# qwerfdsaplking/SATrans

Hardware: AMD Instinct MI355X
Metric: training samples/sec (AliCCP-shaped, emb=32, 3L/4H, meta_mode=QK) (higher is better)
Workload: dtype f32; 1 GPU; BASELINE configs[1]: AliCCP-shaped SATrans training step, 19 fields, 6,571,961 table rows (841 MB fp32), uniform ids, dropout on, dense-Adam+L2 semantics over all rows; batch_per_gpu=8192, global_batch=8192, embedding_dim=32, layers=3, heads=4, fields=19, parallelism=dp1

## Files before the change

include/satrans_hip.h:

```cpp
#ifndef SATRANS_HIP_H
#define SATRANS_HIP_H

#include <stdint.h>

#ifdef __cplusplus
extern "C" {
#endif

#define SATRANS_ABI_VERSION 7

#define SATRANS_OK 0
#define SATRANS_E_BADARG (-1)
#define SATRANS_E_UNSUPPORTED (-2)
#define SATRANS_E_LAUNCH (-3)
#define SATRANS_E_WORKSPACE (-4)

#define SATRANS_ID_F32 0
#define SATRANS_ID_I32 1
#define SATRANS_ID_I64 2

#define SATRANS_META_Q 1
#define SATRANS_META_K 2
#define SATRANS_RELU_OUT 4
#define SATRANS_NO_RES 8
// ... 697 lines not shown
int satrans_layer_bwd_head_supported(const satrans_layer_desc* d, const satrans_head_desc* h);
int satrans_stack_fwd_bf16_head(int n, const satrans_layer_desc* const* descs, const satrans_head_desc* h, void* stream);
int64_t satrans_layer_bwd_head_scratch_floats(const satrans_layer_desc* d, int n_dense);
int satrans_layer_bwd_head(const satrans_layer_desc* d, const satrans_head_desc* h, float* dx, float* slabs, float* g_wq,
                           float* g_wk, float* g_wv, float* g_wo, float* g_ln, float* g_lnq, float* g_lnk, float* g_tab_q,
                           float* g_tab_k, void* stream);

typedef struct satrans_layer_grads {
    float *g_wq, *g_wk, *g_wv, *g_wo, *g_ln, *g_lnq, *g_lnk, *g_tab_q, *g_tab_k;
} satrans_layer_grads;
int satrans_layer_bwd_deferred_supported(const satrans_layer_desc* d);
int satrans_layer_bwd_launch(const satrans_layer_desc* d, const float* dy, float* dx, float* slabs, void* stream);
int satrans_layer_bwd_head_launch(const satrans_layer_desc* d, const satrans_head_desc* h, float* dx, float* slabs, void* stream);
int satrans_layer_bwd_reduce(int n, const satrans_layer_desc* const* h_descs, float* const* h_slabs,
                             const satrans_layer_grads* h_grads, const satrans_head_desc* head, void* stream);

#define SATRANS_OPT_SGD 1
#define SATRANS_OPT_ADAGRAD 2
#define SATRANS_OPT_RMSPROP 3
int satrans_optim_flat(int kind, float* p, const float* g, float* state, int64_t n, float lr, float alpha, float eps, void* stream);
int64_t satrans_head_scratch_floats(int B, int FD, int n_dense);

#define SATRANS_ADAM_EXACT 0
#define SATRANS_ADAM_FAST  1
typedef struct satrans_adam_hparams {
    float lr_over_bc1;
    float bc2_sqrt;
    float beta1, beta2, eps;
    float l2;
    int32_t arith;
// ... 113 lines not shown
```

satrans_amd/csrc/embed_adam.hip:

```cpp
#include <algorithm>
#include <cstdlib>
#include <cstring>

#include <rocprim/rocprim.hpp>

#include "common.h"

namespace satrans {

constexpr int kChunk = 16;
constexpr int kStreamBlock = 256;
constexpr int kStreamBlocks = 2048;

struct AdamK {
    float neg_step, w1, beta2, w2, eps, l2x2, l2;
    double rbc2;
    float rbc2f;
    int fast;
};

__host__ inline AdamK make_adamk(const satrans_adam_hparams& h) {
    AdamK k;
    k.neg_step = -h.lr_over_bc1;
    k.rbc2 = 1.0 / (double)h.bc2_sqrt;
// ... 110 lines not shown
    if (i >= n) return;
    keys[i] = (uint32_t)rows[i];
    pos[i] = (int32_t)i;
}

__global__ void mark_heads_kernel(const int32_t* __restrict__ sorted_rows, int64_t n, uint32_t* __restrict__ touched) {
    const int64_t i = (int64_t)blockIdx.x * blockDim.x + threadIdx.x;
    if (i >= n) return;
    const uint32_t r = (uint32_t)sorted_rows[i];
    if (i > 0 && (uint32_t)sorted_rows[i - 1] == r) return;
    atomicOr(&touched[r >> 5], 1u << (r & 31));
}

constexpr int kSuper = 16;
template <int LPR>
__device__ __forceinline__ void touched_super_body(int64_t group, int q, int64_t chunks, const float4* partial, const int32_t* info,
                                                   const int32_t* trail_row, float4* partial2, int32_t* info2, int32_t* trail_row2,
                                                   float4* done_sum, int32_t* done_row) {
    const int64_t c0 = group * kSuper;
    if (c0 < chunks) {
        const int64_t c1 = min(chunks, c0 + (int64_t)kSuper);
        int f[kSuper];
        float4 lead[kSuper];
#pragma unroll
        for (int u = 0; u < kSuper; ++u) f[u] = c0 + u < c1 ? info[c0 + u] : 0;
#pragma unroll
        for (int u = 0; u < kSuper; ++u)
            lead[u] = c0 + u < c1 ? partial[((c0 + u) * 2 + 0) * LPR + q] : make_float4(0.f, 0.f, 0.f, 0.f);
        bool open = f[0] & 2, is_lead = open;
        int flags2 = open ? 2 : 0;
        int32_t row = -1;
        float4 acc = make_float4(0.f, 0.f, 0.f, 0.f);
#pragma unroll
        for (int u = 0; u < kSuper; ++u) {
            const int64_t c = c0 + u;
            int32_t ended = -1;
            if (f[u] & 2) {
                const float4 g = lead[u];
                acc.x += g.x; acc.y += g.y; acc.z += g.z; acc.w += g.w;
                if (f[u] & 4) {
                    if (is_lead) {
                        partial2[(group * 2 + 0) * LPR + q] = acc;
                        flags2 |= 4;
                    } else {
                        done_sum[c * LPR + q] = acc;
                        ended = row;
                    }
                    open = false;
                    is_lead = false;
                }
            }
            if (f[u] & 1) {
                acc = partial[(c * 2 + 1) * LPR + q];
                row = trail_row[c];
                open = true;
                is_lead = false;
            }
            if (q == 0 && c < c1) done_row[c] = ended;
        }
        if (open) {
            if (is_lead) {
                partial2[(group * 2 + 0) * LPR + q] = acc;
            } else {
                partial2[(group * 2 + 1) * LPR + q] = acc;
                flags2 |= 1;
                if (q == 0) trail_row2[group] = row;
            }
        }
        if (q == 0) info2[group] = flags2;
    }
}

template <int LPR>
__global__ __launch_bounds__(256) void touched_super_kernel(int64_t chunks, const float4* partial, const int32_t* info,
                                                           const int32_t* trail_row, float4* partial2, int32_t* info2,
                                                           int32_t* trail_row2, float4* done_sum, int32_t* done_row) {
    __builtin_amdgcn_s_setprio(3);
    touched_super_body<LPR>(((int64_t)blockIdx.x * 256 + threadIdx.x) / LPR, threadIdx.x % LPR, chunks, partial, info, trail_row, partial2,
                            info2, trail_row2, done_sum, done_row);
}

template <int LPR>
__global__ __launch_bounds__(256) void touched_chunks_kernel(float4* __restrict__ P, float4* __restrict__ M,
                                                            float4* __restrict__ V, const int32_t* __restrict__ sorted_rows,
                                                            const int32_t* __restrict__ src, int64_t n,
                                                            const float4* __restrict__ gemb, float4* partial,
                                                            int32_t* info, int32_t* trail_row,
                                                            float4* __restrict__ rowsum, int32_t* __restrict__ head_of,
                                                            float4* partial2, int32_t* info2, int32_t* trail_row2,
                                                            float4* done_sum, int32_t* done_row) {
    __builtin_amdgcn_s_setprio(3);
    const int64_t group = ((int64_t)blockIdx.x * 256 + threadIdx.x) / LPR;
    const int q = threadIdx.x % LPR;
    const int64_t start = group * kChunk;
    if (start < n) {
        int64_t head = start;
        const int64_t end = min(n, start + (int64_t)kChunk);
        const int32_t prev_row = start > 0 ? sorted_rows[start - 1] : -1;
        const int32_t next_row = end < n ? sorted_rows[end] : -1;
        int32_t cur = sorted_rows[start];
        bool begins = cur != prev_row;
        int flags = 0;
        float4 acc = make_float4(0.f, 0.f, 0.f, 0.f);
        auto flush = [&](bool ends) {
            const bool complete = begins && ends;
            if (q == 0) head_of[head] = complete ? 1 : 0;
            if (complete) {
                rowsum[head * LPR + q] = acc;
            } else if (!begins) {
                partial[(group * 2 + 0) * LPR + q] = acc;
                flags |= 2 | (ends ? 4 : 0);
            } else {
                partial[(group * 2 + 1) * LPR + q] = acc;
                flags |= 1;
                if (q == 0) trail_row[group] = cur;
            }
        };
        constexpr int kBatch = 16;
        for (int64_t jb = start; jb < end; jb += kBatch) {
            int32_t r[kBatch];
            float4 g[kBatch];
#pragma unroll
            for (int u = 0; u < kBatch; ++u) {
                const int64_t j = jb + u;
                const bool ok = j < end;
                r[u] = ok ? sorted_rows[j] : -2;
                const int32_t sidx = ok ? src[j] : 0;
                g[u] = ok ? gemb[(int64_t)sidx * LPR + q] : make_float4(0.f, 0.f, 0.f, 0.f);
            }
#pragma unroll
            for (int u = 0; u < kBatch; ++u) {
                if (jb + u < end) {
                    if (r[u] != cur) {
                        flush(true);
                        cur = r[u];
                        begins = true;
                        head = jb + u;
                        acc = make_float4(0.f, 0.f, 0.f, 0.f);
                    }
                    if (q == 0 && jb + u != head) head_of[jb + u] = 0;
                    acc.x += g[u].x; acc.y += g[u].y; acc.z += g[u].z; acc.w += g[u].w;
                }
            }
        }
        flush(next_row != cur);
        if (q == 0) info[group] = flags;
    }
    constexpr int kGroups = 256 / LPR;
    if constexpr (kGroups % kSuper == 0) {
        __syncthreads();
        const int sg = threadIdx.x / LPR;
        if (sg < kGroups / kSuper)
            touched_super_body<LPR>((int64_t)blockIdx.x * (kGroups / kSuper) + sg, q, (n + kChunk - 1) / kChunk, partial, info, trail_row,
                                    partial2, info2, trail_row2, done_sum, done_row);
    }
}

template <int LPR>
__device__ __forceinline__ void touched_apply_body(int64_t bid, double* s_red, float4* __restrict__ P, float4* __restrict__ M,
                                                   float4* __restrict__ V, const int32_t* __restrict__ sorted_rows,
                                                   int64_t n, const float4* __restrict__ rowsum,
                                                   const int32_t* __restrict__ head_of, const AdamK& k,
                                                   double* __restrict__ reg_partials, float4* __restrict__ G,
                                                   int32_t* __restrict__ last, int t) {
    const int64_t j = (bid * 256 + threadIdx.x) / LPR;
    const int q = threadIdx.x % LPR;
    double reg = 0.0;
    if (j < n && head_of[j] == 1) {
        const int64_t at = (int64_t)sorted_rows[j] * LPR + q;
// ... 1356 lines not shown
```

satrans_amd/csrc/layer_fused.hip:

```cpp
#include <hip/hip_ext.h>

#include "layer_fused_common.h"

namespace satrans {

struct KernelTimer {
    static constexpr int kPairs = 512;
    struct Pair { hipEvent_t start, stop; int kind; };
    Pair pairs[kPairs];
    int made = 0, used = 0;
    bool armed = false;
    Pair* next(int kind) {
        if (!armed || used >= kPairs) return nullptr;
        if (used >= made) {
            if (hipEventCreate(&pairs[made].start) != hipSuccess || hipEventCreate(&pairs[made].stop) != hipSuccess) return nullptr;
            ++made;
        }
        pairs[used].kind = kind;
        return &pairs[used++];
    }
};
static KernelTimer g_ktimer;

#ifdef SATRANS_DIAG_FWDSAVE
// ... 1665 lines not shown
            }
            if (threadIdx.x == 0) {
                float gb = 0.f, lsum = 0.f;
                for (int ls = 0; ls < Tsamp; ++ls) { lsum += s_fin[ls]; gb += s_fin[64 + ls]; }
                prow[ncol] = gb;
                prow[ncol + 1] = lsum;
            }
        }
    }
}


#undef WGRAD
constexpr int kRG = kReduceGroups;
constexpr int kReduceMaxLayers = 8;
__device__ __forceinline__ void fused_common_reduce(const float* __restrict__ common, int G, int D, int flags, int block,
                                                    float* g_wq, float* g_wk, float* g_wv, float* g_wo, float* g_ln,
                                                    float* g_lnq, float* g_lnk) {
    __shared__ float s_a[kRG][32], s_b[kRG][32];
    const int CSZ = 4 * D * D + 6 * D, DD = D * D;
    const int lane = threadIdx.x & 31, grp = threadIdx.x >> 5;
    const int e = block * 32 + lane;
    const bool plain = !(flags & (SATRANS_GATE | SATRANS_BILINEAR));
    const bool mq = plain && (flags & SATRANS_META_Q) && g_lnq, mk = plain && (flags & SATRANS_META_K) && g_lnk;
    const bool shared = mq && mk && g_lnq == g_lnk;
    const int r = e - 4 * DD;
    const bool second = shared && r >= 2 * D && r < 4 * D;
    const int share = (G + kRG - 1) / kRG;
    const int lo = grp * share, hi = min(G, lo + share);
    float acc = 0.f, acc2 = 0.f;
    if (e < CSZ) {
#pragma unroll 4
        for (int w = lo; w < hi; ++w) {
            acc += common[(size_t)w * CSZ + e];
            if (second) acc2 += common[(size_t)w * CSZ + e + 2 * D];
        }
    }
    s_a[grp][lane] = acc;
    s_b[grp][lane] = acc2;
    __syncthreads();
    if (grp != 0 || e >= CSZ) return;
    float t = 0.f, t2 = 0.f;
    for (int k = 0; k < kRG; ++k) { t += s_a[k][lane]; t2 += s_b[k][lane]; }
    if (e < DD) { g_wq[e] += t; return; }
    if (e < 2 * DD) { g_wk[e - DD] += t; return; }
    if (e < 3 * DD) { g_wv[e - 2 * DD] += t; return; }
    if (e < 4 * DD) { g_wo[e - 3 * DD] += t; return; }
    if (r < 2 * D) { g_ln[r] += t; return; }
    if (r < 4 * D) {
        if (shared) g_lnq[r - 2 * D] += t + t2;
        else if (mq) g_lnq[r - 2 * D] += t;
        return;
    }
    if (mk && !shared) g_lnk[r - 4 * D] += t;
}

__device__ __forceinline__ void fused_records_reduce(int n_layers, const float* const* records_of, float* const* g_tab_q_of,
                                                     float* const* g_tab_k_of, const int32_t* __restrict__ seg,
                                                     int S, int T, int G, int D, int U, int H, int flags, int64_t tab_stride,
                                                     int block, int s) {
    __shared__ float s_q[kRG][32], s_k[kRG][32];
    const int TSZ = 4 * D * U, d = D / H;
    const bool gate = flags & SATRANS_GATE, bil = flags & SATRANS_BILINEAR;
    const int half = gate ? D : (bil ? D * d : 2 * D * U);
    const int lane = threadIdx.x & 31, grp = threadIdx.x >> 5;
    const int e = block * 32 + lane;
    int total = 0, pre = 0;
    for (int k = 0; k < S; ++k) {
        if (k == s) pre = total;
        total += tiles_of(seg, k, T);
    }
    const int nt = tiles_of(seg, s, T);
    if (nt == 0) return;
    const int per = (total + G - 1) / G;
    const int w_lo = pre / per, w_hi = (pre + nt - 1) / per;
    const int share = (w_hi - w_lo + kRG) / kRG;
    const int a = w_lo + grp * share, b = min(w_hi + 1, a + share);
    const bool mq = bil || (flags & SATRANS_META_Q), mk = !bil && (flags & SATRANS_META_K);
    int src_q = e, src_k = half + e;
    if (bil && e < half) {
        const int h = e / (d * d), i = (e / d) % d, j = e % d;
        src_q = (h * d + i) * D + h * d + j;
    }
    float aq[kReduceMaxLayers], ak[kReduceMaxLayers];
#pragma unroll
    for (int l = 0; l < kReduceMaxLayers; ++l) {
        aq[l] = 0.f; ak[l] = 0.f;
        if (l < n_layers && e < half) {
            const float* records = records_of[l];
#pragma unroll 4
            for (int w = a; w < b; ++w) {
                const float* rec = records + (size_t)(w + s) * TSZ;
                if (mq) aq[l] += rec[src_q];
                if (mk) ak[l] += rec[src_k];
            }
        }
    }
#pragma unroll
    for (int l = 0; l < kReduceMaxLayers; ++l) {
        if (l >= n_layers) break;
        s_q[grp][lane] = aq[l];
        s_k[grp][lane] = ak[l];
        __syncthreads();
        if (grp == 0 && e < half) {
            float tq = 0.f, tk = 0.f;
            for (int k = 0; k < kRG; ++k) { tq += s_q[k][lane]; tk += s_k[k][lane]; }
            float* g_tab_q = g_tab_q_of[l];
            float* g_tab_k = g_tab_k_of[l];
            if (mq && mk && g_tab_q == g_tab_k) {
                g_tab_q[(size_t)s * tab_stride + e] += tq + tk;
            } else {
                if (mq) g_tab_q[(size_t)s * tab_stride + e] += tq;
                if (mk) g_tab_k[(size_t)s * tab_stride + e] += tk;
            }
        }
        __syncthreads();
    }
}

__global__ __launch_bounds__(32 * kRG) void fused_reduce_kernel(const float* __restrict__ common, const float* __restrict__ records,
                                                         const int32_t* __restrict__ seg, int S, int T, int G, int D, int U,
                                                         int H, int flags, int64_t tab_stride, int common_blocks, int record_blocks,
                                                         float* g_wq, float* g_wk, float* g_wv, float* g_wo, float* g_ln,
                                                         float* g_lnq, float* g_lnk, float* g_tab_q, float* g_tab_k) {
    const int bx = blockIdx.x;
    if (bx < common_blocks) {
        fused_common_reduce(common, G, D, flags, bx, g_wq, g_wk, g_wv, g_wo, g_ln, g_lnq, g_lnk);
    } else {
        const int rb = bx - common_blocks;
        const float* recs[1] = {records};
        float *gq[1] = {g_tab_q}, *gk[1] = {g_tab_k};
        fused_records_reduce(1, recs, gq, gk, seg, S, T, G, D, U, H, flags, tab_stride, rb % record_blocks, rb / record_blocks);
    }
}

struct ReduceLayers {
    int n;
    const float* slabs[kReduceMaxLayers];
    float* g[kReduceMaxLayers][9];
};
struct ReduceHead {
    const float* partial;
    int nblk, ncol;
    float *g_w, *g_b;
    double* loss_sum;
};
__device__ __forceinline__ void head_partials_reduce(const ReduceHead& hd, int block) {
    __shared__ double s_acc[kRG][32];
    const int lane = threadIdx.x & 31, grp = threadIdx.x >> 5;
    const int c = block * 32 + lane, ncol = hd.ncol;
    const int share = (hd.nblk + kRG - 1) / kRG;
    const int lo = grp * share, hi = min(hd.nblk, lo + share);
    double acc = 0.0;
    if (c < ncol + 2) {
        if (c == ncol + 1) {
            for (int k = lo; k < hi; ++k) acc += (double)hd.partial[(size_t)k * (ncol + 2) + c];
        } else {
            float a32 = 0.f;
#pragma unroll 8
            for (int k = lo; k < hi; ++k) a32 += hd.partial[(size_t)k * (ncol + 2) + c];
            acc = (double)a32;
        }
    }
    s_acc[grp][lane] = acc;
    __syncthreads();
    if (grp != 0 || c >= ncol + 2) return;
    if (c == ncol + 1) {
        double t = 0.0;
        for (int k = 0; k < kRG; ++k) t += s_acc[k][lane];
        hd.loss_sum[0] += t;
        return;
    }
    float t = 0.f;
    for (int k = 0; k < kRG; ++k) t += (float)s_acc[k][lane];
    if (c < ncol) hd.g_w[c] += t;
    else hd.g_b[0] += t;
}
__global__ __launch_bounds__(32 * kRG) void fused_reduce_all_kernel(ReduceLayers R, ReduceHead hd, const int32_t* __restrict__ seg,
                                                             int S, int T, int G, int D, int U, int H, int flags,
                                                             int64_t tab_stride, int common_blocks, int record_blocks,
                                                             int per_layer) {
    __builtin_amdgcn_s_setprio(3);
    int bx = blockIdx.x;
    if (bx < R.n * common_blocks) {
        const int l = bx / common_blocks;
        float* const* g = R.g[l];
        fused_common_reduce(R.slabs[l], G, D, flags, bx - l * common_blocks, g[0], g[1], g[2], g[3], g[4], g[5], g[6]);
        return;
    }
    bx -= R.n * common_blocks;
    const int n_rec = per_layer - common_blocks;
    if (bx < n_rec) {
        const float* recs[kReduceMaxLayers];
        float *gq[kReduceMaxLayers], *gk[kReduceMaxLayers];
        for (int l = 0; l < R.n; ++l) {
            recs[l] = R.slabs[l] + (size_t)G * (4 * D * D + 6 * D);
            gq[l] = R.g[l][7];
            gk[l] = R.g[l][8];
        }
        fused_records_reduce(R.n, recs, gq, gk, seg, S, T, G, D, U, H, flags, tab_stride, bx % record_blocks, bx / record_blocks);
        return;
    }
    head_partials_reduce(hd, bx - n_rec);
}


static int fused_bwd_ft(const satrans_layer_desc* d) {
    if (d->D != 32 || d->H != 4) return 0;
    const bool same = d->tab_q == d->tab_k && d->lnq_g == d->lnk_g && d->lnq_b == d->lnk_b;
    const int mod = (d->flags & SATRANS_GATE) ? 1 : ((d->flags & SATRANS_BILINEAR) ? 2 : 0);
    if (mod) return same && d->F == 19 ? 19 : 0;
    return same ? (d->F == 19 ? 19 : 0) : (d->F == 15 ? 15 : 0);
}
#ifdef SATRANS_HANDOVER_LDS
static bool fused_save_rows(const satrans_layer_desc* d) { return false; }
#else
static bool fused_save_rows(const satrans_layer_desc* d) { return kAttnMfma && fused_bwd_ft(d) != 0; }
#endif
// ... 165 lines not shown
    if (fused_bwd_plan(d, p)) {
        const int64_t CSZ = 4 * (int64_t)d->D * d->D + 6 * d->D, TSZ = 4 * (int64_t)d->D * fused_width(d);
        n = std::max<int64_t>(n, (int64_t)p.G * CSZ + (int64_t)(p.G + d->S) * TSZ);
    }
    return n;
}

static int launch_fused_reduce(const satrans_layer_desc* d, const FusedBwdPlan& p, float* slabs, float* g_wq, float* g_wk,
                               float* g_wv, float* g_wo, float* g_ln, float* g_lnq, float* g_lnk, float* g_tab_q, float* g_tab_k,
                               hipStream_t stream) {
    const int D = d->D, U = fused_width(d), CSZ = 4 * D * D + 6 * D;
    float* records = slabs + (size_t)p.G * CSZ;
    const bool meta = d->flags & (SATRANS_META_Q | SATRANS_META_K | SATRANS_BILINEAR);
    const int row_elems = (d->flags & SATRANS_GATE) ? D : ((d->flags & SATRANS_BILINEAR) ? D * (D / d->H) : 2 * D * U);
    SATRANS_REQUIRE(!meta || g_tab_q, SATRANS_E_BADARG, "layer_bwd: null generated-row gradient");
    const int common_blocks = (int)ceil_div(CSZ, 32), record_blocks = (int)ceil_div(row_elems, 32);
    fused_reduce_kernel<<<(unsigned)(common_blocks + (meta ? record_blocks * d->S : 0)), 32 * kRG, 0, stream>>>(
        slabs, records, d->seg, d->S, p.T, p.G, D, U, d->H, d->flags, d->tab_stride, common_blocks, record_blocks, g_wq, g_wk, g_wv,
        g_wo, g_ln, g_lnq, g_lnk, g_tab_q, g_tab_k);
    SATRANS_CHECK_LAUNCH("fused_reduce_kernel");
    return SATRANS_OK;
}

extern "C" int satrans_layer_bwd_launch_fused(const satrans_layer_desc* d, const float* dy, float* dx, float* slabs, void* stream_) {
    hipStream_t stream = (hipStream_t)stream_;
    FusedBwdPlan p;
    SATRANS_REQUIRE(dy && dx && slabs, SATRANS_E_BADARG, "layer_bwd: null pointer");
    const bool same = d->tab_q == d->tab_k && d->lnq_g == d->lnk_g && d->lnq_b == d->lnk_b;
    int rc;
    {
    SATRANS_REQUIRE(fused_bwd_plan(d, p), SATRANS_E_UNSUPPORTED, "layer_bwd(fused): shape not built");
    SATRANS_REQUIRE((int64_t)d->B * d->F < ((int64_t)1 << 31), SATRANS_E_UNSUPPORTED, "layer_bwd(fused): B * F must stay below 2^31");
// ... 110 lines not shown
}

extern "C" int satrans_layer_bwd_head_fused(const satrans_layer_desc* d, const satrans_head_desc* h, float* dx, float* slabs,
                                            float* g_wq, float* g_wk, float* g_wv, float* g_wo, float* g_ln, float* g_lnq,
                                            float* g_lnk, float* g_tab_q, float* g_tab_k, void* stream_) {
    SATRANS_REQUIRE(g_wq && g_wk && g_wv && g_wo && g_ln && h->loss_sum && h->g_w && h->g_b, SATRANS_E_BADARG, "layer_bwd_head: null pointer");
    int rc = satrans_layer_bwd_head_launch_fused(d, h, dx, slabs, stream_);
    if (rc) return rc;
    FusedBwdPlan p;
    fused_bwd_plan(d, p, true);
    rc = launch_fused_reduce(d, p, slabs, g_wq, g_wk, g_wv, g_wo, g_ln, g_lnq, g_lnk, g_tab_q, g_tab_k, (hipStream_t)stream_);
    if (rc) return rc;
    return satrans_head_reduce_partials(h->scratch, p.G, d->F * d->D + h->n_dense, h->g_w, h->g_b, h->loss_sum, stream_);
}

extern "C" int satrans_layer_bwd_reduce_fused(int n, const satrans_layer_desc* const* descs, float* const* slabs,
                                              const satrans_layer_grads* grads, const satrans_head_desc* head, void* stream_) {
    hipStream_t stream = (hipStream_t)stream_;
    SATRANS_REQUIRE(n >= 1 && n <= kReduceMaxLayers && descs && slabs && grads, SATRANS_E_BADARG, "layer_bwd_reduce: 1..%d layers", kReduceMaxLayers);
    const satrans_layer_desc* d = descs[0];
    FusedBwdPlan p;
    SATRANS_REQUIRE(fused_bwd_plan(d, p), SATRANS_E_UNSUPPORTED, "layer_bwd_reduce: shape not built");
    const int D = d->D, U = fused_width(d), CSZ = 4 * D * D + 6 * D;
    const bool meta = d->flags & (SATRANS_META_Q | SATRANS_META_K | SATRANS_BILINEAR);
    const int row_elems = (d->flags & SATRANS_GATE) ? D : ((d->flags & SATRANS_BILINEAR) ? D * (D / d->H) : 2 * D * U);
    const int common_blocks = (int)ceil_div(CSZ, 32), record_blocks = (int)ceil_div(row_elems, 32);
    const int per_layer = common_blocks + (meta ? record_blocks * d->S : 0);
    ReduceLayers R;
    R.n = n;
    for (int l = 0; l < n; ++l) {
        const satrans_layer_desc* e = descs[l];
        FusedBwdPlan q;
        SATRANS_REQUIRE(e->B == d->B && e->F == d->F && e->D == d->D && e->U == d->U && e->H == d->H && e->S == d->S &&
                        e->flags == d->flags && e->seg == d->seg && e->tab_stride == d->tab_stride && fused_bwd_plan(e, q) &&
                        q.G == p.G && q.T == p.T, SATRANS_E_BADARG, "layer_bwd_reduce: layer %d differs from layer 0 in shape, flags or bucketing", l);
        const satrans_layer_grads& g = grads[l];
        SATRANS_REQUIRE(slabs[l] && g.g_wq && g.g_wk && g.g_wv && g.g_wo && g.g_ln && (!meta || g.g_tab_q), SATRANS_E_BADARG,
                        "layer_bwd_reduce: null pointer (layer %d)", l);
        R.slabs[l] = slabs[l];
        float* gp[9] = {g.g_wq, g.g_wk, g.g_wv, g.g_wo, g.g_ln, g.g_lnq, g.g_lnk, g.g_tab_q, g.g_tab_k};
        for (int k = 0; k < 9; ++k) R.g[l][k] = gp[k];
    }
    ReduceHead hd{};
    int head_blocks = 0;
    if (head) {
        SATRANS_REQUIRE(head->scratch && head->g_w && head->g_b && head->loss_sum, SATRANS_E_BADARG, "layer_bwd_reduce: null head pointer");
        FusedBwdPlan ph;
        SATRANS_REQUIRE(fused_bwd_plan(d, ph, true), SATRANS_E_UNSUPPORTED, "layer_bwd_reduce: fused head not built for this shape");
        hd.partial = head->scratch; hd.nblk = ph.G; hd.ncol = d->F * d->D + head->n_dense;
        hd.g_w = head->g_w; hd.g_b = head->g_b; hd.loss_sum = head->loss_sum;
        head_blocks = (int)ceil_div(hd.ncol + 2, 32);
    }
    fused_reduce_all_kernel<<<(unsigned)(n * common_blocks + (per_layer - common_blocks) + head_blocks), 32 * kRG, 0, stream>>>(
        R, hd, d->seg, d->S, p.T, p.G, D, U, d->H, d->flags, d->tab_stride, common_blocks, record_blocks, per_layer);
    SATRANS_CHECK_LAUNCH("fused_reduce_all_kernel");
    return SATRANS_OK;
}

#ifdef SATRANS_STAMPS
extern "C" int satrans_debug_read_stamps(unsigned long long* h_out, int reset) {
    if (hipMemcpyFromSymbol(h_out, HIP_SYMBOL(satrans::g_stamps), sizeof(unsigned long long) * 16) != hipSuccess) return -1;
    if (reset) {
        unsigned long long z[16] = {0};
        if (hipMemcpyToSymbol(HIP_SYMBOL(satrans::g_stamps), z, sizeof(z)) != hipSuccess) return -1;
    }
    return 0;
}
#endif

extern "C" int satrans_kernel_timing(int on) {
    const int was = satrans::g_ktimer.armed ? 1 : 0;
// ... 25 lines not shown
```

satrans_amd/native.py:

```python
from __future__ import annotations

import ctypes as C
import os
import subprocess
from typing import Optional

import torch

os.environ.setdefault("GPU_MAX_HW_QUEUES", "8")

_HERE = os.path.dirname(os.path.abspath(__file__))
LIB_PATH = os.environ.get("SATRANS_LIB_PATH") or os.path.join(_HERE, "libsatrans_hip.so")
ABI_VERSION = 7

ID_F32, ID_I32, ID_I64 = 0, 1, 2
META_Q, META_K, RELU_OUT, NO_RES, TRAIN, GATE, BILINEAR = 1, 2, 4, 8, 16, 32, 64
X_SORTED, Y_SORTED = 128, 256

_c_f32p = C.c_void_p
_vp = C.c_void_p


class LayerDesc(C.Structure):
    _fields_ = [
# ... 492 lines not shown
                                           C.POINTER(HeadDesc), _vp]),
    "satrans_head_scratch_floats": (C.c_int64, [C.c_int, C.c_int, C.c_int]),
    "satrans_head": (C.c_int, [_vp, _vp, C.c_int64, _vp, C.c_int, C.c_int, C.c_int, _vp, _vp, _vp, _vp, _vp, _vp,
                               _vp, _vp, _vp, _vp, _vp]),
"satrans_head_loss": (C.c_int, [_vp, _vp, C.c_int64, _vp, C.c_int, C.c_int, C.c_int, _vp, _vp, _vp, _vp, _vp, _vp,
                                    _vp, _vp, _vp, _vp, C.c_int, _vp]),
    "satrans_point_loss_partials": (C.c_int64, [C.c_int]),
    "satrans_point_loss": (C.c_int, [_vp, C.c_int64, _vp, C.c_int, C.c_int, C.c_int, _vp, _vp, _vp, _vp, _vp]),
    "satrans_optim_flat": (C.c_int, [C.c_int, _vp, _vp, _vp, C.c_int64, C.c_float, C.c_float, C.c_float, _vp]),
    "satrans_adam_flat": (C.c_int, [_vp, _vp, _vp, _vp, C.c_int64, C.POINTER(AdamHParams), _vp]),
    "satrans_adam_flat_sum": (C.c_int, [_vp, _vp, _vp, _vp, C.c_int64, C.POINTER(AdamHParams), _vp, C.c_int64, _vp, _vp]),
    "satrans_embed_sort_workspace_bytes": (C.c_int64, [C.c_int64, C.c_int64]),
    "satrans_embed_sort": (C.c_int, [_vp, C.c_int64, C.c_int64, _vp, _vp, _vp, _vp, C.c_int64, _vp, _vp]),
    "satrans_embed_reg_partials": (C.c_int64, [C.c_int64, C.c_int64, C.c_int]),
    "satrans_embed_partial_ws_floats": (C.c_int64, [C.c_int64, C.c_int]),
    "satrans_scenario_table_fwd": (C.c_int, [_vp, _vp, _vp, C.c_int, C.c_int, C.c_int, _vp, _vp]),
    "satrans_scenario_table_bwd_ws_floats": (C.c_int64, [C.c_int, C.c_int]),
    "satrans_scenario_table_bwd": (C.c_int, [_vp, _vp, _vp, C.c_int, C.c_int, C.c_int, _vp, _vp, _vp, _vp, _vp]),
    "satrans_scenario_inputs_fwd": (C.c_int, [C.POINTER(_vp), _vp, C.c_int, C.c_int, C.c_int, _vp, _vp, C.c_int, _vp, _vp]),
    "satrans_scenario_inputs_bwd": (C.c_int, [C.POINTER(_vp), C.POINTER(C.c_int32), _vp, C.c_int, C.c_int, C.c_int, _vp, _vp,
                                              _vp, C.c_int, _vp]),
    "satrans_scenario_relu_fwd": (C.c_int, [_vp, C.c_int64, _vp, _vp]),
    "satrans_scenario_relu_bwd": (C.c_int, [_vp, _vp, C.c_int64, _vp, _vp]),
    "satrans_embed_adam_touched": (C.c_int, [_vp, _vp, _vp, C.c_int, _vp, _vp, C.c_int64, _vp, _vp,
                                             C.POINTER(AdamHParams), _vp, _vp, C.c_int, _vp]),
    "satrans_embed_adam_untouched": (C.c_int, [_vp, _vp, _vp, C.c_int64, C.c_int64, C.c_int, _vp, C.POINTER(AdamHParams),
                                               _vp, C.c_int, _vp]),
    "satrans_embed_mark_touched": (C.c_int, [_vp, C.c_int64, C.c_int64, _vp, _vp]),
    "satrans_embed_segment_sums": (C.c_int, [_vp, _vp, C.c_int64, _vp, C.c_int, _vp, _vp, _vp, _vp]),
    "satrans_embed_adam_rows_partials": (C.c_int64, [C.c_int64, C.c_int]),
# ... 124 lines not shown
```

Baseline: 9.045 million samples/s.

## Vectorize bwd gradient reductions with float4 loads and stage chunk partials in LDS

The fused backward reduce kernels now use wave-wide (64-lane) columns with float4 loads, batched multi-row loads and multi-layer record accumulation held in shared LDS buffers. The previous 32-wide scalar loads are replaced. The embedding touched-chunks kernel preloads all sorted rows, source ids and gradients of a chunk up front. Its in-block super-walk reads partials from shared memory instead of re-reading global memory. A new reduce_slabs entry point is also exposed that takes explicit G/T. The aim is more memory-level parallelism and fewer global round trips, at the cost of more registers and LDS and a new 16-byte alignment requirement.

```diff
diff --git a/include/satrans_hip.h b/include/satrans_hip.h
--- a/include/satrans_hip.h
+++ b/include/satrans_hip.h
@@ -735,6 +735,9 @@
 int satrans_layer_bwd_head_launch(const satrans_layer_desc* d, const satrans_head_desc* h, float* dx, float* slabs, void* stream);
 int satrans_layer_bwd_reduce(int n, const satrans_layer_desc* const* h_descs, float* const* h_slabs,
                              const satrans_layer_grads* h_grads, const satrans_head_desc* head, void* stream);
+int satrans_layer_bwd_reduce_slabs(int n, const satrans_layer_desc* const* descs, int G, int T, float* const* slabs,
+                                   const satrans_layer_grads* grads, const satrans_head_desc* head, int head_rows, int per_layer,
+                                   void* stream);
 
 #define SATRANS_OPT_SGD 1
 #define SATRANS_OPT_ADAGRAD 2
diff --git a/satrans_amd/csrc/embed_adam.hip b/satrans_amd/csrc/embed_adam.hip
--- a/satrans_amd/csrc/embed_adam.hip
+++ b/satrans_amd/csrc/embed_adam.hip
@@ -148,8 +148,8 @@
 
 constexpr int kSuper = 16;
 template <int LPR>
-__device__ __forceinline__ void touched_super_body(int64_t group, int q, int64_t chunks, const float4* partial, const int32_t* info,
-                                                   const int32_t* trail_row, float4* partial2, int32_t* info2, int32_t* trail_row2,
+__device__ __forceinline__ void touched_super_body(int64_t group, int q, int64_t chunks, int64_t base, const float4* partial,
+                                                   const int32_t* info, const int32_t* trail_row, float4* partial2, int32_t* info2, int32_t* trail_row2,
                                                    float4* done_sum, int32_t* done_row) {
     const int64_t c0 = group * kSuper;
     if (c0 < chunks) {
@@ -157,10 +157,10 @@
         int f[kSuper];
         float4 lead[kSuper];
 #pragma unroll
-        for (int u = 0; u < kSuper; ++u) f[u] = c0 + u < c1 ? info[c0 + u] : 0;
+        for (int u = 0; u < kSuper; ++u) f[u] = c0 + u < c1 ? info[c0 + u - base] : 0;
 #pragma unroll
         for (int u = 0; u < kSuper; ++u)
-            lead[u] = c0 + u < c1 ? partial[((c0 + u) * 2 + 0) * LPR + q] : make_float4(0.f, 0.f, 0.f, 0.f);
+            lead[u] = c0 + u < c1 ? partial[((c0 + u - base) * 2 + 0) * LPR + q] : make_float4(0.f, 0.f, 0.f, 0.f);
         bool open = f[0] & 2, is_lead = open;
         int flags2 = open ? 2 : 0;
         int32_t row = -1;
@@ -185,8 +185,8 @@
                 }
             }
             if (f[u] & 1) {
-                acc = partial[(c * 2 + 1) * LPR + q];
-                row = trail_row[c];
+                acc = partial[((c - base) * 2 + 1) * LPR + q];
+                row = trail_row[c - base];
                 open = true;
                 is_lead = false;
             }
@@ -210,7 +210,7 @@
                                                            const int32_t* trail_row, float4* partial2, int32_t* info2,
                                                            int32_t* trail_row2, float4* done_sum, int32_t* done_row) {
     __builtin_amdgcn_s_setprio(3);
-    touched_super_body<LPR>(((int64_t)blockIdx.x * 256 + threadIdx.x) / LPR, threadIdx.x % LPR, chunks, partial, info, trail_row, partial2,
+    touched_super_body<LPR>(((int64_t)blockIdx.x * 256 + threadIdx.x) / LPR, threadIdx.x % LPR, chunks, 0, partial, info, trail_row, partial2,
                             info2, trail_row2, done_sum, done_row);
 }
 
@@ -224,16 +224,30 @@
                                                             float4* partial2, int32_t* info2, int32_t* trail_row2,
                                                             float4* done_sum, int32_t* done_row) {
     __builtin_amdgcn_s_setprio(3);
+    constexpr int kGroups = 256 / LPR;
+    constexpr bool kWalk = kGroups % kSuper == 0;
+    __shared__ float4 s_partial[kWalk ? kGroups * 2 * LPR : 1];
+    __shared__ int32_t s_info[kWalk ? kGroups : 1], s_trail_row[kWalk ? kGroups : 1];
+    const int lg = threadIdx.x / LPR;
     const int64_t group = ((int64_t)blockIdx.x * 256 + threadIdx.x) / LPR;
     const int q = threadIdx.x % LPR;
     const int64_t start = group * kChunk;
     if (start < n) {
         int64_t head = start;
         const int64_t end = min(n, start + (int64_t)kChunk);
-        const int32_t prev_row = start > 0 ? sorted_rows[start - 1] : -1;
-        const int32_t next_row = end < n ? sorted_rows[end] : -1;
-        int32_t cur = sorted_rows[start];
-        bool begins = cur != prev_row;
+        int32_t r[kChunk], sidx[kChunk];
+        float4 g[kChunk];
+#pragma unroll
+        for (int u = 0; u < kChunk; ++u) {
+            const int64_t j = min(start + u, end - 1);
+            r[u] = sorted_rows[j];
+            sidx[u] = src[j];
+        }
+        const int32_t prev_row = sorted_rows[max(start - 1, (int64_t)0)], next_row = sorted_rows[min(end, n - 1)];
+#pragma unroll
+        for (int u = 0; u < kChunk; ++u) g[u] = gemb[(int64_t)sidx[u] * LPR + q];
+        int32_t cur = r[0];
+        bool begins = start == 0 || cur != prev_row;
         int flags = 0;
         float4 acc = make_float4(0.f, 0.f, 0.f, 0.f);
         auto flush = [&](bool ends) {
@@ -243,50 +257,43 @@
                 rowsum[head * LPR + q] = acc;
             } else if (!begins) {
                 partial[(group * 2 + 0) * LPR + q] = acc;
+                if constexpr (kWalk) s_partial[(lg * 2 + 0) * LPR + q] = acc;
                 flags |= 2 | (ends ? 4 : 0);
             } else {
                 partial[(group * 2 + 1) * LPR + q] = acc;
+                if constexpr (kWalk) s_partial[(lg * 2 + 1) * LPR + q] = acc;
                 flags |= 1;
-                if (q == 0) trail_row[group] = cur;
+                if (q == 0) {
+                    trail_row[group] = cur;
+                    if constexpr (kWalk) s_trail_row[lg] = cur;
+                }
             }
         };
-        constexpr int kBatch = 16;
-        for (int64_t jb = start; jb < end; jb += kBatch) {
-            int32_t r[kBatch];
-            float4 g[kBatch];
-#pragma unroll
-            for (int u = 0; u < kBatch; ++u) {
-                const int64_t j = jb + u;
-                const bool ok = j < end;
-                r[u] = ok ? sorted_rows[j] : -2;
-                const int32_t sidx = ok ? src[j] : 0;
-                g[u] = ok ? gemb[(int64_t)sidx * LPR + q] : make_float4(0.f, 0.f, 0.f, 0.f);
+#pragma unroll
+        for (int u = 0; u < kChunk; ++u) {
+            if (start + u < end) {
+                if (r[u] != cur) {
+                    flush(true);
+                    cur = r[u];
+                    begins = true;
+                    head = start + u;
+                    acc = make_float4(0.f, 0.f, 0.f, 0.f);
+                }
+                if (q == 0 && start + u != head) head_of[start + u] = 0;
+                acc.x += g[u].x; acc.y += g[u].y; acc.z += g[u].z; acc.w += g[u].w;
             }
-#pragma unroll
-            for (int u = 0; u < kBatch; ++u) {
-                if (jb + u < end) {
-                    if (r[u] != cur) {
-                        flush(true);
-                        cur = r[u];
-                        begins = true;
-                        head = jb + u;
-                        acc = make_float4(0.f, 0.f, 0.f, 0.f);
-                    }
-                    if (q == 0 && jb + u != head) head_of[jb + u] = 0;
-                    acc.x += g[u].x; acc.y += g[u].y; acc.z += g[u].z; acc.w += g[u].w;
-                }
-            }
-        }
-        flush(next_row != cur);
-        if (q == 0) info[group] = flags;
-    }
-    constexpr int kGroups = 256 / LPR;
-    if constexpr (kGroups % kSuper == 0) {
+        }
+        flush(end == n || next_row != cur);
+        if (q == 0) {
+            info[group] = flags;
+            if constexpr (kWalk) s_info[lg] = flags;
+        }
+    }
+    if constexpr (kWalk) {
         __syncthreads();
-        const int sg = threadIdx.x / LPR;
-        if (sg < kGroups / kSuper)
-            touched_super_body<LPR>((int64_t)blockIdx.x * (kGroups / kSuper) + sg, q, (n + kChunk - 1) / kChunk, partial, info, trail_row,
-                                    partial2, info2, trail_row2, done_sum, done_row);
+        if (lg < kGroups / kSuper)
+            touched_super_body<LPR>((int64_t)blockIdx.x * (kGroups / kSuper) + lg, q, (n + kChunk - 1) / kChunk, (int64_t)blockIdx.x * kGroups,
+                                    s_partial, s_info, s_trail_row, partial2, info2, trail_row2, done_sum, done_row);
     }
 }
 
diff --git a/satrans_amd/csrc/layer_fused.hip b/satrans_amd/csrc/layer_fused.hip
--- a/satrans_amd/csrc/layer_fused.hip
+++ b/satrans_amd/csrc/layer_fused.hip
@@ -1703,34 +1703,72 @@
 #undef WGRAD
 constexpr int kRG = kReduceGroups;
 constexpr int kReduceMaxLayers = 8;
-__device__ __forceinline__ void fused_common_reduce(const float* __restrict__ common, int G, int D, int flags, int block,
+constexpr int kRE = 4 * kWave;
+constexpr int kRU = 8;
+constexpr int kReduceThreads = kWave * kRG;
+constexpr int kReduceLdsFloats = 2 * kRG * kRE;
+
+__device__ __forceinline__ float4 reduce_ld4(const float* p) { return *reinterpret_cast<const float4*>(p); }
+__device__ __forceinline__ void reduce_add4(float4& a, const float4& b) { a.x += b.x; a.y += b.y; a.z += b.z; a.w += b.w; }
+
+template <int kW, typename LoadA, typename LoadB>
+__device__ __forceinline__ void reduce_ordered_sum(float4& acc_a, float4& acc_b, int lo, int hi, bool do_a, bool do_b, LoadA load_a,
+                                                   LoadB load_b) {
+    const float4 zero = make_float4(0.f, 0.f, 0.f, 0.f);
+    for (int w0 = lo; w0 < hi; w0 += kW) {
+        float4 va[kW], vb[kW];
+#pragma unroll
+        for (int u = 0; u < kW; ++u) {
+            const int w = min(w0 + u, hi - 1);
+            va[u] = do_a ? load_a(w) : zero;
+            vb[u] = do_b ? load_b(w) : zero;
+        }
+#pragma unroll
+        for (int u = 0; u < kW; ++u) {
+            if (w0 + u < hi) {
+                if (do_a) reduce_add4(acc_a, va[u]);
+                if (do_b) reduce_add4(acc_b, vb[u]);
+            }
+        }
+    }
+}
+
+__device__ __forceinline__ void fused_common_reduce(float* s_lds, const float* __restrict__ common, int G, int D, int flags, int block,
                                                     float* g_wq, float* g_wk, float* g_wv, float* g_wo, float* g_ln,
                                                     float* g_lnq, float* g_lnk) {
-    __shared__ float s_a[kRG][32], s_b[kRG][32];
+    float* s_a = s_lds;
+    float* s_b = s_lds + kRG * kRE;
     const int CSZ = 4 * D * D + 6 * D, DD = D * D;
-    const int lane = threadIdx.x & 31, grp = threadIdx.x >> 5;
-    const int e = block * 32 + lane;
+    const int lane = threadIdx.x & (kWave - 1), grp = threadIdx.x / kWave;
     const bool plain = !(flags & (SATRANS_GATE | SATRANS_BILINEAR));
     const bool mq = plain && (flags & SATRANS_META_Q) && g_lnq, mk = plain && (flags & SATRANS_META_K) && g_lnk;
     const bool shared = mq && mk && g_lnq == g_lnk;
-    const int r = e - 4 * DD;
-    const bool second = shared && r >= 2 * D && r < 4 * D;
     const int share = (G + kRG - 1) / kRG;
     const int lo = grp * share, hi = min(G, lo + share);
-    float acc = 0.f, acc2 = 0.f;
-    if (e < CSZ) {
-#pragma unroll 4
-        for (int w = lo; w < hi; ++w) {
-            acc += common[(size_t)w * CSZ + e];
-            if (second) acc2 += common[(size_t)w * CSZ + e + 2 * D];
-        }
-    }
-    s_a[grp][lane] = acc;
-    s_b[grp][lane] = acc2;
+    {
+        const int e4 = block * kRE + 4 * lane;
+        const int r4 = e4 - 4 * DD;
+        const bool second4 = shared && r4 >= 2 * D && r4 < 4 * D;
+        float4 acc = make_float4(0.f, 0.f, 0.f, 0.f), acc2 = acc;
+        if (e4 < CSZ) {
+            const float* col = common + e4;
+            if (__any(second4))
+                reduce_ordered_sum<kRU>(acc, acc2, lo, hi, true, true, [&](int w) { return reduce_ld4(col + (size_t)w * CSZ); },
+                                   [&](int w) { return second4 ? reduce_ld4(col + (size_t)w * CSZ + 2 * D) : make_float4(0.f, 0.f, 0.f, 0.f); });
+            else
+                reduce_ordered_sum<2 * kRU>(acc, acc2, lo, hi, true, false, [&](int w) { return reduce_ld4(col + (size_t)w * CSZ); },
+                                   [&](int) { return make_float4(0.f, 0.f, 0.f, 0.f); });
+        }
+        if (!second4) acc2 = make_float4(0.f, 0.f, 0.f, 0.f);
+        *reinterpret_cast<float4*>(&s_a[grp * kRE + 4 * lane]) = acc;
+        *reinterpret_cast<float4*>(&s_b[grp * kRE + 4 * lane]) = acc2;
+    }
     __syncthreads();
-    if (grp != 0 || e >= CSZ) return;
+    const int col = threadIdx.x, e = block * kRE + col;
+    if (col >= kRE || e >= CSZ) return;
+    const int r = e - 4 * DD;
     float t = 0.f, t2 = 0.f;
-    for (int k = 0; k < kRG; ++k) { t += s_a[k][lane]; t2 += s_b[k][lane]; }
+    for (int k = 0; k < kRG; ++k) { t += s_a[k * kRE + col]; t2 += s_b[k * kRE + col]; }
     if (e < DD) { g_wq[e] += t; return; }
     if (e < 2 * DD) { g_wk[e - DD] += t; return; }
     if (e < 3 * DD) { g_wv[e - 2 * DD] += t; return; }
@@ -1744,16 +1782,18 @@
     if (mk && !shared) g_lnk[r - 4 * D] += t;
 }
 
-__device__ __forceinline__ void fused_records_reduce(int n_layers, const float* const* records_of, float* const* g_tab_q_of,
-                                                     float* const* g_tab_k_of, const int32_t* __restrict__ seg,
-                                                     int S, int T, int G, int D, int U, int H, int flags, int64_t tab_stride,
-                                                     int block, int s) {
-    __shared__ float s_q[kRG][32], s_k[kRG][32];
+template <typename RecordsOf, typename TabQOf, typename TabKOf>
+__device__ __forceinline__ void fused_records_reduce(float* s_lds, int n_layers, RecordsOf records_of, TabQOf g_tab_q_of,
+                                                     TabKOf g_tab_k_of, const int32_t* __restrict__ seg, int S, int T, int G, int D, int U, int H,
+                                                     int flags, int64_t tab_stride, int block, int s) {
+    float* s_q = s_lds;
+    float* s_k = s_lds + kRG * kRE;
     const int TSZ = 4 * D * U, d = D / H;
     const bool gate = flags & SATRANS_GATE, bil = flags & SATRANS_BILINEAR;
     const int half = gate ? D : (bil ? D * d : 2 * D * U);
-    const int lane = threadIdx.x & 31, grp = threadIdx.x >> 5;
-    const int e = block * 32 + lane;
+    const int lane = threadIdx.x & (kWave - 1), grp = threadIdx.x / kWave;
+    const int e4 = block * kRE + 4 * lane;
+    const int col = threadIdx.x, e = block * kRE + col;
     int total = 0, pre = 0;
     for (int k = 0; k < S; ++k) {
         if (k == s) pre = total;
@@ -1766,36 +1806,60 @@
     const int share = (w_hi - w_lo + kRG) / kRG;
     const int a = w_lo + grp * share, b = min(w_hi + 1, a + share);
     const bool mq = bil || (flags & SATRANS_META_Q), mk = !bil && (flags & SATRANS_META_K);
-    int src_q = e, src_k = half + e;
-    if (bil && e < half) {
-        const int h = e / (d * d), i = (e / d) % d, j = e % d;
-        src_q = (h * d + i) * D + h * d + j;
-    }
-    float aq[kReduceMaxLayers], ak[kReduceMaxLayers];
-#pragma unroll
-    for (int l = 0; l < kReduceMaxLayers; ++l) {
-        aq[l] = 0.f; ak[l] = 0.f;
-        if (l < n_layers && e < half) {
-            const float* records = records_of[l];
-#pragma unroll 4
-            for (int w = a; w < b; ++w) {
-                const float* rec = records + (size_t)(w + s) * TSZ;
-                if (mq) aq[l] += rec[src_q];
-                if (mk) ak[l] += rec[src_k];
-            }
-        }
-    }
-#pragma unroll
-    for (int l = 0; l < kReduceMaxLayers; ++l) {
-        if (l >= n_layers) break;
-        s_q[grp][lane] = aq[l];
-        s_k[grp][lane] = ak[l];
+    int src_q[4];
+#pragma unroll
+    for (int i4 = 0; i4 < 4; ++i4) {
+        const int eb = min(e4 + i4, half - 1);
+        const int h = eb / (d * d), i = (eb / d) % d, j = eb % d;
+        src_q[i4] = bil ? (h * d + i) * D + h * d + j : eb;
+    }
+    constexpr int kRL = 4, kWR = 2;
+    const float4 zero = make_float4(0.f, 0.f, 0.f, 0.f);
+    for (int l0 = 0; l0 < n_layers; l0 += kRL) {
+    float4 aq[kRL], ak[kRL];
+    const float* records[kRL];
+#pragma unroll
+    for (int l = 0; l < kRL; ++l) {
+        aq[l] = zero; ak[l] = zero;
+        records[l] = records_of(min(l0 + l, n_layers - 1)) + (size_t)s * TSZ;
+    }
+    if (e4 < half) {
+        for (int w0 = a; w0 < b; w0 += kWR) {
+            float4 vq[kRL][kWR], vk[kRL][kWR];
+#pragma unroll
+            for (int l = 0; l < kRL; ++l) {
+#pragma unroll
+                for (int u = 0; u < kWR; ++u) {
+                    const float* rec = records[l] + (size_t)min(w0 + u, b - 1) * TSZ;
+                    const bool on = l0 + l < n_layers;
+                    vq[l][u] = !(on && mq) ? zero
+                               : bil ? make_float4(rec[src_q[0]], rec[src_q[1]], rec[src_q[2]], rec[src_q[3]]) : reduce_ld4(rec + e4);
+                    vk[l][u] = on && mk ? reduce_ld4(rec + half + e4) : zero;
+                }
+            }
+#pragma unroll
+            for (int l = 0; l < kRL; ++l) {
+#pragma unroll
+                for (int u = 0; u < kWR; ++u) {
+                    if (w0 + u < b && l0 + l < n_layers) {
+                        if (mq) reduce_add4(aq[l], vq[l][u]);
+                        if (mk) reduce_add4(ak[l], vk[l][u]);
+                    }
+                }
+            }
+        }
+    }
+#pragma unroll
+    for (int l = 0; l < kRL; ++l) {
+        if (l0 + l >= n_layers) break;
+        *reinterpret_cast<float4*>(&s_q[grp * kRE + 4 * lane]) = aq[l];
+        *reinterpret_cast<float4*>(&s_k[grp * kRE + 4 * lane]) = ak[l];
         __syncthreads();
-        if (grp == 0 && e < half) {
+        if (col < kRE && e < half) {
             float tq = 0.f, tk = 0.f;
-            for (int k = 0; k < kRG; ++k) { tq += s_q[k][lane]; tk += s_k[k][lane]; }
-            float* g_tab_q = g_tab_q_of[l];
-            float* g_tab_k = g_tab_k_of[l];
+            for (int k = 0; k < kRG; ++k) { tq += s_q[k * kRE + col]; tk += s_k[k * kRE + col]; }
+            float* g_tab_q = g_tab_q_of(l0 + l);
+            float* g_tab_k = g_tab_k_of(l0 + l);
             if (mq && mk && g_tab_q == g_tab_k) {
                 g_tab_q[(size_t)s * tab_stride + e] += tq + tk;
             } else {
@@ -1805,21 +1869,21 @@
         }
         __syncthreads();
     }
-}
-
-__global__ __launch_bounds__(32 * kRG) void fused_reduce_kernel(const float* __restrict__ common, const float* __restrict__ records,
+    }
+}
+
+__global__ __launch_bounds__(kReduceThreads) void fused_reduce_kernel(const float* __restrict__ common, const float* __restrict__ records,
                                                          const int32_t* __restrict__ seg, int S, int T, int G, int D, int U,
                                                          int H, int flags, int64_t tab_stride, int common_blocks, int record_blocks,
                                                          float* g_wq, float* g_wk, float* g_wv, float* g_wo, float* g_ln,
                                                          float* g_lnq, float* g_lnk, float* g_tab_q, float* g_tab_k) {
+    __shared__ __align__(16) float s_lds[kReduceLdsFloats];
     const int bx = blockIdx.x;
     if (bx < common_blocks) {
-        fused_common_reduce(common, G, D, flags, bx, g_wq, g_wk, g_wv, g_wo, g_ln, g_lnq, g_lnk);
+        fused_common_reduce(s_lds, common, G, D, flags, bx, g_wq, g_wk, g_wv, g_wo, g_ln, g_lnq, g_lnk);
     } else {
         const int rb = bx - common_blocks;
-        const float* recs[1] = {records};
-        float *gq[1] = {g_tab_q}, *gk[1] = {g_tab_k};
-        fused_records_reduce(1, recs, gq, gk, seg, S, T, G, D, U, H, flags, tab_stride, rb % record_blocks, rb / record_blocks);
+        fused_records_reduce(s_lds, 1, [&](int) { return records; }, [&](int) { return g_tab_q; }, [&](int) { return g_tab_k; }, seg, S, T, G, D, U, H, flags, tab_stride, rb % record_blocks, rb / record_blocks);
     }
 }
 
@@ -1834,10 +1898,11 @@
     float *g_w, *g_b;
     double* loss_sum;
 };
-__device__ __forceinline__ void head_partials_reduce(const ReduceHead& hd, int block) {
-    __shared__ double s_acc[kRG][32];
-    const int lane = threadIdx.x & 31, grp = threadIdx.x >> 5;
-    const int c = block * 32 + lane, ncol = hd.ncol;
+__device__ __forceinline__ void head_partials_reduce(float* s_lds, const ReduceHead& hd, int block) {
+    static_assert(kRG * kWave * sizeof(double) <= kReduceLdsFloats * sizeof(float), "the head's group sums fit the LDS array");
+    double (*s_acc)[kWave] = reinterpret_cast<double (*)[kWave]>(s_lds);
+    const int lane = threadIdx.x & (kWave - 1), grp = threadIdx.x / kWave;
+    const int c = block * kWave + lane, ncol = hd.ncol;
     const int share = (hd.nblk + kRG - 1) / kRG;
     const int lo = grp * share, hi = min(hd.nblk, lo + share);
     double acc = 0.0;
@@ -1865,32 +1930,27 @@
     if (c < ncol) hd.g_w[c] += t;
     else hd.g_b[0] += t;
 }
-__global__ __launch_bounds__(32 * kRG) void fused_reduce_all_kernel(ReduceLayers R, ReduceHead hd, const int32_t* __restrict__ seg,
+__global__ __launch_bounds__(kReduceThreads) void fused_reduce_all_kernel(ReduceLayers R, ReduceHead hd, const int32_t* __restrict__ seg,
                                                              int S, int T, int G, int D, int U, int H, int flags,
                                                              int64_t tab_stride, int common_blocks, int record_blocks,
                                                              int per_layer) {
     __builtin_amdgcn_s_setprio(3);
+    __shared__ __align__(16) float s_lds[kReduceLdsFloats];
     int bx = blockIdx.x;
     if (bx < R.n * common_blocks) {
         const int l = bx / common_blocks;
         float* const* g = R.g[l];
-        fused_common_reduce(R.slabs[l], G, D, flags, bx - l * common_blocks, g[0], g[1], g[2], g[3], g[4], g[5], g[6]);
+        fused_common_reduce(s_lds, R.slabs[l], G, D, flags, bx - l * common_blocks, g[0], g[1], g[2], g[3], g[4], g[5], g[6]);
         return;
     }
     bx -= R.n * common_blocks;
     const int n_rec = per_layer - common_blocks;
     if (bx < n_rec) {
-        const float* recs[kReduceMaxLayers];
-        float *gq[kReduceMaxLayers], *gk[kReduceMaxLayers];
-        for (int l = 0; l < R.n; ++l) {
-            recs[l] = R.slabs[l] + (size_t)G * (4 * D * D + 6 * D);
-            gq[l] = R.g[l][7];
-            gk[l] = R.g[l][8];
-        }
-        fused_records_reduce(R.n, recs, gq, gk, seg, S, T, G, D, U, H, flags, tab_stride, bx % record_blocks, bx / record_blocks);
+        fused_records_reduce(s_lds, R.n, [&](int l) { return R.slabs[l] + (size_t)G * (4 * D * D + 6 * D); },
+                             [&](int l) { return R.g[l][7]; }, [&](int l) { return R.g[l][8]; }, seg, S, T, G, D, U, H, flags, tab_stride, bx % record_blocks, bx / record_blocks);
         return;
     }
-    head_partials_reduce(hd, bx - n_rec);
+    head_partials_reduce(s_lds, hd, bx - n_rec);
 }
 
 
@@ -2086,8 +2146,9 @@
     const bool meta = d->flags & (SATRANS_META_Q | SATRANS_META_K | SATRANS_BILINEAR);
     const int row_elems = (d->flags & SATRANS_GATE) ? D : ((d->flags & SATRANS_BILINEAR) ? D * (D / d->H) : 2 * D * U);
     SATRANS_REQUIRE(!meta || g_tab_q, SATRANS_E_BADARG, "layer_bwd: null generated-row gradient");
-    const int common_blocks = (int)ceil_div(CSZ, 32), record_blocks = (int)ceil_div(row_elems, 32);
-    fused_reduce_kernel<<<(unsigned)(common_blocks + (meta ? record_blocks * d->S : 0)), 32 * kRG, 0, stream>>>(
+    SATRANS_REQUIRE((uintptr_t)slabs % 16 == 0, SATRANS_E_BADARG, "layer_bwd: the slab buffer must be 16-byte aligned");
+    const int common_blocks = (int)ceil_div(CSZ, kRE), record_blocks = (int)ceil_div(row_elems, kRE);
+    fused_reduce_kernel<<<(unsigned)(common_blocks + (meta ? record_blocks * d->S : 0)), kReduceThreads, 0, stream>>>(
         slabs, records, d->seg, d->S, p.T, p.G, D, U, d->H, d->flags, d->tab_stride, common_blocks, record_blocks, g_wq, g_wk, g_wv,
         g_wo, g_ln, g_lnq, g_lnk, g_tab_q, g_tab_k);
     SATRANS_CHECK_LAUNCH("fused_reduce_kernel");
@@ -2228,29 +2289,26 @@
     return satrans_head_reduce_partials(h->scratch, p.G, d->F * d->D + h->n_dense, h->g_w, h->g_b, h->loss_sum, stream_);
 }
 
-extern "C" int satrans_layer_bwd_reduce_fused(int n, const satrans_layer_desc* const* descs, float* const* slabs,
-                                              const satrans_layer_grads* grads, const satrans_head_desc* head, void* stream_) {
-    hipStream_t stream = (hipStream_t)stream_;
-    SATRANS_REQUIRE(n >= 1 && n <= kReduceMaxLayers && descs && slabs && grads, SATRANS_E_BADARG, "layer_bwd_reduce: 1..%d layers", kReduceMaxLayers);
+static int launch_fused_reduce_all(int n, const satrans_layer_desc* const* descs, int G, int T, float* const* slabs,
+                                   const satrans_layer_grads* grads, const satrans_head_desc* head, int head_rows,
+                                   hipStream_t stream) {
     const satrans_layer_desc* d = descs[0];
-    FusedBwdPlan p;
-    SATRANS_REQUIRE(fused_bwd_plan(d, p), SATRANS_E_UNSUPPORTED, "layer_bwd_reduce: shape not built");
     const int D = d->D, U = fused_width(d), CSZ = 4 * D * D + 6 * D;
     const bool meta = d->flags & (SATRANS_META_Q | SATRANS_META_K | SATRANS_BILINEAR);
     const int row_elems = (d->flags & SATRANS_GATE) ? D : ((d->flags & SATRANS_BILINEAR) ? D * (D / d->H) : 2 * D * U);
-    const int common_blocks = (int)ceil_div(CSZ, 32), record_blocks = (int)ceil_div(row_elems, 32);
+    const int common_blocks = (int)ceil_div(CSZ, kRE), record_blocks = (int)ceil_div(row_elems, kRE);
     const int per_layer = common_blocks + (meta ? record_blocks * d->S : 0);
     ReduceLayers R;
     R.n = n;
     for (int l = 0; l < n; ++l) {
         const satrans_layer_desc* e = descs[l];
-        FusedBwdPlan q;
         SATRANS_REQUIRE(e->B == d->B && e->F == d->F && e->D == d->D && e->U == d->U && e->H == d->H && e->S == d->S &&
-                        e->flags == d->flags && e->seg == d->seg && e->tab_stride == d->tab_stride && fused_bwd_plan(e, q) &&
-                        q.G == p.G && q.T == p.T, SATRANS_E_BADARG, "layer_bwd_reduce: layer %d differs from layer 0 in shape, flags or bucketing", l);
+                        e->flags == d->flags && e->seg == d->seg && e->tab_stride == d->tab_stride, SATRANS_E_BADARG,
+                        "layer_bwd_reduce: layer %d differs from layer 0 in shape, flags or bucketing", l);
         const satrans_layer_grads& g = grads[l];
         SATRANS_REQUIRE(slabs[l] && g.g_wq && g.g_wk && g.g_wv && g.g_wo && g.g_ln && (!meta || g.g_tab_q), SATRANS_E_BADARG,
                         "layer_bwd_reduce: null pointer (layer %d)", l);
+        SATRANS_REQUIRE((uintptr_t)slabs[l] % 16 == 0, SATRANS_E_BADARG, "layer_bwd_reduce: slab buffer %d must be 16-byte aligned", l);
         R.slabs[l] = slabs[l];
         float* gp[9] = {g.g_wq, g.g_wk, g.g_wv, g.g_wo, g.g_ln, g.g_lnq, g.g_lnk, g.g_tab_q, g.g_tab_k};
         for (int k = 0; k < 9; ++k) R.g[l][k] = gp[k];
@@ -2259,16 +2317,57 @@
     int head_blocks = 0;
     if (head) {
         SATRANS_REQUIRE(head->scratch && head->g_w && head->g_b && head->loss_sum, SATRANS_E_BADARG, "layer_bwd_reduce: null head pointer");
+        hd.partial = head->scratch; hd.nblk = head_rows; hd.ncol = d->F * d->D + head->n_dense;
+        hd.g_w = head->g_w; hd.g_b = head->g_b; hd.loss_sum = head->loss_sum;
+        head_blocks = (int)ceil_div(hd.ncol + 2, kWave);
+    }
+    fused_reduce_all_kernel<<<(unsigned)(n * common_blocks + (per_layer - common_blocks) + head_blocks), kReduceThreads, 0, stream>>>(
+        R, hd, d->seg, d->S, T, G, D, U, d->H, d->flags, d->tab_stride, common_blocks, record_blocks, per_layer);
+    SATRANS_CHECK_LAUNCH("fused_reduce_all_kernel");
+    return SATRANS_OK;
+}
+
+extern "C" int satrans_layer_bwd_reduce_fused(int n, const satrans_layer_desc* const* descs, float* const* slabs,
+                                              const satrans_layer_grads* grads, const satrans_head_desc* head, void* stream_) {
+    SATRANS_REQUIRE(n >= 1 && n <= kReduceMaxLayers && descs && slabs && grads, SATRANS_E_BADARG, "layer_bwd_reduce: 1..%d layers", kReduceMaxLayers);
+    const satrans_layer_desc* d = descs[0];
+    FusedBwdPlan p;
+    SATRANS_REQUIRE(fused_bwd_plan(d, p), SATRANS_E_UNSUPPORTED, "layer_bwd_reduce: shape not built");
+    for (int l = 1; l < n; ++l) {
+        FusedBwdPlan q;
+        SATRANS_REQUIRE(descs[l]->B == d->B && descs[l]->F == d->F && descs[l]->S == d->S && fused_bwd_plan(descs[l], q) && q.G == p.G &&
+                        q.T == p.T, SATRANS_E_BADARG, "layer_bwd_reduce: layer %d differs from layer 0 in shape, flags or bucketing", l);
+    }
+    int head_rows = 0;
+    if (head) {
         FusedBwdPlan ph;
         SATRANS_REQUIRE(fused_bwd_plan(d, ph, true), SATRANS_E_UNSUPPORTED, "layer_bwd_reduce: fused head not built for this shape");
-        hd.partial = head->scratch; hd.nblk = ph.G; hd.ncol = d->F * d->D + head->n_dense;
-        hd.g_w = head->g_w; hd.g_b = head->g_b; hd.loss_sum = head->loss_sum;
-        head_blocks = (int)ceil_div(hd.ncol + 2, 32);
-    }
-    fused_reduce_all_kernel<<<(unsigned)(n * common_blocks + (per_layer - common_blocks) + head_blocks), 32 * kRG, 0, stream>>>(
-        R, hd, d->seg, d->S, p.T, p.G, D, U, d->H, d->flags, d->tab_stride, common_blocks, record_blocks, per_layer);
-    SATRANS_CHECK_LAUNCH("fused_reduce_all_kernel");
-    return SATRANS_OK;
+        head_rows = ph.G;
+    }
+    return launch_fused_reduce_all(n, descs, p.G, p.T, slabs, grads, head, head_rows, (hipStream_t)stream_);
+}
+
+extern "C" int satrans_layer_bwd_reduce_slabs(int n, const satrans_layer_desc* const* descs, int G, int T, float* const* slabs,
+                                              const satrans_layer_grads* grads, const satrans_head_desc* head, int head_rows,
+                                              int per_layer, void* stream_) {
+    SATRANS_REQUIRE(n >= 1 && n <= kReduceMaxLayers && descs && slabs && grads, SATRANS_E_BADARG, "layer_bwd_reduce_slabs: 1..%d layers", kReduceMaxLayers);
+    SATRANS_REQUIRE(G >= 1 && T >= 1 && (!head || head_rows >= 1), SATRANS_E_BADARG, "layer_bwd_reduce_slabs: G, T and head_rows must be positive");
+    for (int l = 0; l < n; ++l)
+        SATRANS_REQUIRE(descs[l] && descs[l]->seg && satrans_layer_fused_supported(descs[l]) && descs[l]->D <= 32, SATRANS_E_UNSUPPORTED,
+                        "layer_bwd_reduce_slabs: shape not built (layer %d)", l);
+    if (!per_layer) return launch_fused_reduce_all(n, descs, G, T, slabs, grads, head, head_rows, (hipStream_t)stream_);
+    FusedBwdPlan p{};
+    p.G = G; p.T = T;
+    for (int l = 0; l < n; ++l) {
+        const satrans_layer_grads& g = grads[l];
+        SATRANS_REQUIRE(slabs[l] && g.g_wq && g.g_wk && g.g_wv && g.g_wo && g.g_ln, SATRANS_E_BADARG, "layer_bwd_reduce_slabs: null pointer (layer %d)", l);
+        int rc = launch_fused_reduce(descs[l], p, slabs[l], g.g_wq, g.g_wk, g.g_wv, g.g_wo, g.g_ln, g.g_lnq, g.g_lnk, g.g_tab_q, g.g_tab_k,
+                                     (hipStream_t)stream_);
+        if (rc) return rc;
+    }
+    if (!head) return SATRANS_OK;
+    return satrans_head_reduce_partials(head->scratch, head_rows, descs[0]->F * descs[0]->D + head->n_dense, head->g_w, head->g_b,
+                                        head->loss_sum, stream_);
 }
 
 #ifdef SATRANS_STAMPS
diff --git a/satrans_amd/native.py b/satrans_amd/native.py
--- a/satrans_amd/native.py
+++ b/satrans_amd/native.py
@@ -530,6 +530,8 @@
     "satrans_embed_sort": (C.c_int, [_vp, C.c_int64, C.c_int64, _vp, _vp, _vp, _vp, C.c_int64, _vp, _vp]),
     "satrans_embed_reg_partials": (C.c_int64, [C.c_int64, C.c_int64, C.c_int]),
     "satrans_embed_partial_ws_floats": (C.c_int64, [C.c_int64, C.c_int]),
+    "satrans_layer_bwd_reduce_slabs": (C.c_int, [C.c_int, C.POINTER(C.POINTER(LayerDesc)), C.c_int, C.c_int, C.POINTER(_vp),
+                                                 C.POINTER(LayerGrads), C.POINTER(HeadDesc), C.c_int, C.c_int, _vp]),
     "satrans_scenario_table_fwd": (C.c_int, [_vp, _vp, _vp, C.c_int, C.c_int, C.c_int, _vp, _vp]),
     "satrans_scenario_table_bwd_ws_floats": (C.c_int64, [C.c_int, C.c_int]),
     "satrans_scenario_table_bwd": (C.c_int, [_vp, _vp, _vp, C.c_int, C.c_int, C.c_int, _vp, _vp, _vp, _vp, _vp]),
```

Result: no change. 9.127 million samples/s, median of 6 (+0.9%).
